# s-esposito/MonoGS

Hardware: AMD Instinct MI355X
Metric: rasteriser fwd+bwd Mpix/s @1080p (higher is better)
Workload: dtype f32; 1 GPU; C5: 2000000 Gaussians, 1920x1080, fwd+bwd, seeded synthetic map (SURVEY.md 8d), one keyframe per GPU; gaussians=2000000, width=1920, height=1080, settle_steps=60, instance_count=device-side (capacity mode, overflow checked), parallelism=keyframe-per-gpu x1

## Files before the change

monogs_amd/csrc/blend.hip:

```cpp
#include "common.h"
#include "tile_sort.h"

#include <type_traits>


namespace mgs {

#ifdef BS_TRACE
static unsigned long long* g_trace_fwd = nullptr;
static unsigned long long* g_trace_bwd = nullptr;
static unsigned long long g_trace_bwd_records = 0;
#define BS_STAMP(v) asm volatile("s_memrealtime %0\n\ts_waitcnt lgkmcnt(0)" : "=s"(v) :: "memory")
#endif

__device__ __forceinline__ uint32_t bcast(uint32_t v, int lane) {
    return (uint32_t)__builtin_amdgcn_readlane((int)v, lane);
}

constexpr int MGS_WG_WAVES = 4;
#define MGS_TILE_WAVE(ntiles_, tile_, wave_, ws_)                                                   \
    const int tile_ = (int)blockIdx.x, wave_ = __builtin_amdgcn_readfirstlane((int)(threadIdx.x >> 6)), ws_ = wave_; \
    if (tile_ >= (ntiles_)) return;
struct BlendArgs {
#ifdef BS_TRACE
    unsigned long long* trace;
#endif
    const float4* __restrict__ rec;
    const uint32_t* __restrict__ point_list;
    const uint2* __restrict__ ranges;
    const float* __restrict__ bg;
    unsigned long long* fwd_masks;
    int W, H, gx;
};
__device__ __forceinline__ size_t fwd_mask_word(uint32_t range_x, int tile, int wave) {
    return ((size_t)(range_x / WAVE) + (size_t)tile) * 4 + (size_t)wave;
}

__device__ __forceinline__ bool quadrant_hit(const float4 c , const float4 n ,
                                             float qx0, float qy0, unsigned long long alive) {
    const float x0 = qx0 - 0.05f - c.x, x1 = qx0 + (float)(SUB - 1) + 0.05f - c.x;
    const float y0 = qy0 - 0.05f - c.y, y1 = qy0 + (float)(SUB - 1) + 0.05f - c.y;
    if (c.z < 0.f) return false;
    if (!((c.z >= x0) && (-c.z <= x1) && (c.w >= y0) && (-c.w <= y1))) return false;
    {
        const int ix0 = (int)fminf(8.f, fmaxf(0.f, ceilf(-x0 - c.z - 0.06f))), ix1 = (int)fminf(7.f, fmaxf(-1.f, floorf(-x0 + c.z + 0.06f)));
        const int iy0 = (int)fminf(8.f, fmaxf(0.f, ceilf(-y0 - c.w - 0.06f))), iy1 = (int)fminf(7.f, fmaxf(-1.f, floorf(-y0 + c.w + 0.06f)));
        if (ix0 > ix1 || iy0 > iy1) return false;
        const unsigned long long cols = (unsigned long long)((0xFFu >> (7 - ix1)) & (0xFFu << ix0) & 0xFFu) * 0x0101010101010101ull;
        const unsigned long long rows = (~0ull >> (8 * (7 - iy1))) & (~0ull << (8 * iy0));
        if ((cols & rows & alive) == 0ull) return false;
    }
    if (x0 <= 0.f && x1 >= 0.f && y0 <= 0.f && y1 >= 0.f) return true;
    if (!(n.x > 0.f) || !(n.z > 0.f)) return true;
    const float rby = -n.y * __builtin_amdgcn_rcpf(n.z), rbx = -n.y * __builtin_amdgcn_rcpf(n.x);
    auto edge_x = [&](float xe) {
        const float t = fminf(y1, fmaxf(y0, rby * xe));
        return n.x * xe * xe + 2.f * n.y * xe * t + n.z * t * t;
    };
    auto edge_y = [&](float ye) {
        const float t = fminf(x1, fmaxf(x0, rbx * ye));
        return n.x * t * t + 2.f * n.y * t * ye + n.z * ye * ye;
    };
    const float qmin = fminf(fminf(edge_x(x0), edge_x(x1)), fminf(edge_y(y0), edge_y(y1)));
    return qmin <= 1.02f;
}

struct Rec {
    float px, py, ca, cb, cc, op, r, g, b, z;
};
__device__ __forceinline__ Rec fetch(const BlendArgs& a, uint32_t gid_uniform) {
    const const_float_p p = MGS_CONST(reinterpret_cast<const float*>(a.rec)) + (size_t)gid_uniform * REC_FLOATS;
    return Rec{p[R_X], p[R_Y], p[R_CA], p[R_CB], p[R_CC], p[R_OPAC], p[R_R], p[R_G], p[R_B], p[R_DEPTH]};
}

template <bool TOUCH>
__device__ __forceinline__ void blend_one(unsigned long long& live, unsigned long long& mask, float& T, uint32_t& last, float& C0, float& C1, float& C2,
                                      float& D, const Rec& g, float power, float alpha, uint32_t pos, int j,
                                      int& touched_cnt) {
    const float test_T = T * (1.f - alpha);
    float w;
    int cnt;
    if (TOUCH) {
        asm volatile(
            "s_mov_b64 exec, %[live]\n\t"
            "v_cmpx_nlt_f32_e32 vcc, 0, %[power]\n\t"
            "v_cmpx_ngt_f32_e32 vcc, %[amin], %[alpha]\n\t"
            "v_cmp_gt_f32_e32 vcc, %[tmin], %[tt]\n\t"
            "s_andn2_b64 exec, exec, vcc\n\t"
            "s_andn2_b64 %[live], %[live], vcc\n\t"
            "s_cselect_b64 %[mask], %[mask], 0\n\t"
            "v_mul_f32_e32 %[w], %[alpha], %[T]\n\t"
            "v_mov_b32_e32 %[T], %[tt]\n\t"
            "v_mov_b32_e32 %[last], %[pos]\n\t"
            "v_cmp_lt_f32_e32 vcc, 0.5, %[tt]\n\t"
            "v_fmac_f32_e32 %[C0], %[cr], %[w]\n\t"
            "v_fmac_f32_e32 %[C1], %[cg], %[w]\n\t"
            "s_bcnt1_i32_b64 %[cnt], vcc\n\t"
            "s_mov_b32 m0, %[j]\n\t"
            "v_fmac_f32_e32 %[C2], %[cb], %[w]\n\t"
            "v_fmac_f32_e32 %[D], %[cz], %[w]\n\t"
            "s_mov_b64 exec, -1\n\t"
            "v_writelane_b32 %[tc], %[cnt], m0\n\t"
            : [live] "+s"(live), [mask] "+s"(mask), [T] "+v"(T), [last] "+v"(last), [C0] "+v"(C0), [C1] "+v"(C1), [C2] "+v"(C2), [D] "+v"(D),
              [w] "=&v"(w), [cnt] "=&s"(cnt), [tc] "+v"(touched_cnt)
            : [power] "v"(power), [alpha] "v"(alpha), [tt] "v"(test_T), [amin] "s"(1.0f / 255.0f), [tmin] "s"(0.0001f),
              [pos] "s"(pos), [cr] "v"(g.r), [cg] "v"(g.g), [cb] "v"(g.b), [cz] "v"(g.z), [j] "s"(j)
            : "vcc", "scc", "m0");
    } else {
        asm volatile(
            "s_mov_b64 exec, %[live]\n\t"
            "v_cmpx_nlt_f32_e32 vcc, 0, %[power]\n\t"
            "v_cmpx_ngt_f32_e32 vcc, %[amin], %[alpha]\n\t"
            "v_cmp_gt_f32_e32 vcc, %[tmin], %[tt]\n\t"
            "s_andn2_b64 exec, exec, vcc\n\t"
            "s_andn2_b64 %[live], %[live], vcc\n\t"
            "s_cselect_b64 %[mask], %[mask], 0\n\t"
            "v_mul_f32_e32 %[w], %[alpha], %[T]\n\t"
            "v_mov_b32_e32 %[T], %[tt]\n\t"
            "v_mov_b32_e32 %[last], %[pos]\n\t"
            "v_fmac_f32_e32 %[C0], %[cr], %[w]\n\t"
            "v_fmac_f32_e32 %[C1], %[cg], %[w]\n\t"
            "v_fmac_f32_e32 %[C2], %[cb], %[w]\n\t"
            "v_fmac_f32_e32 %[D], %[cz], %[w]\n\t"
            "s_mov_b64 exec, -1\n\t"
            : [live] "+s"(live), [mask] "+s"(mask), [T] "+v"(T), [last] "+v"(last), [C0] "+v"(C0), [C1] "+v"(C1), [C2] "+v"(C2), [D] "+v"(D),
              [w] "=&v"(w)
            : [power] "v"(power), [alpha] "v"(alpha), [tt] "v"(test_T), [amin] "s"(1.0f / 255.0f), [tmin] "s"(0.0001f),
              [pos] "s"(pos), [cr] "v"(g.r), [cg] "v"(g.g), [cb] "v"(g.b), [cz] "v"(g.z)
            : "vcc", "scc");
    }
}

template <bool SORT>
__global__ void __launch_bounds__(256) blend_forward_kernel(BlendArgs a, float* __restrict__ out_color,
                                                            float* __restrict__ out_depth,
                                                            float* __restrict__ out_opacity,
                                                            float* __restrict__ final_T,
                                                            uint32_t* __restrict__ n_contrib,
                                                            int32_t* __restrict__ n_touched,
                                                            uint2* ranges_rw ,
                                                            const uint32_t* __restrict__ sort_err,
                                                            uint32_t* __restrict__ status, TileSortArgs ts,
                                                            const unsigned long long* __restrict__ prepare ,
                                                            int P, int lines_per_tile ) {
    MGS_TILE_WAVE(a.gx * ((a.H + TILE - 1) / TILE), tile, wave, ws)
    if (prepare) {
        float* const acc = reinterpret_cast<float*>((uintptr_t)MGS_CONST_U64(prepare)[1]);
        if (acc) {
            const int first = tile * lines_per_tile;
            const int n4 = 4 * min(lines_per_tile, P - first);
            float4* const base = reinterpret_cast<float4*>(acc + (size_t)first * GRAD_FLOATS);
            for (int i = (int)threadIdx.x; i < n4; i += 256) base[i] = make_float4(0.f, 0.f, 0.f, 0.f);
        }
    }
    const int tx = tile % a.gx, ty = tile / a.gx;
    const int lane = threadIdx.x & 63;
    const bool first_of_tile = wave == 0 && lane == 0;
    const int qx0i = tx * TILE + (wave & 1) * SUB, qy0i = ty * TILE + (wave >> 1) * SUB;
    const int pxi = qx0i + (lane & 7), pyi = qy0i + (lane >> 3);
    const bool inside = pxi < a.W && pyi < a.H;
    const float pxf = (float)pxi, pyf = (float)pyi;
    const float qx0 = (float)qx0i, qy0 = (float)qy0i;
    uint2 range = ranges_rw[tile];
    const uint2 range_raw = range;
    const bool sort_bad = sort_err != nullptr && radix_failed(sort_err) != 0u;
    {
        if (sort_bad && tile == 0 && first_of_tile && status) atomicOr(status, (uint32_t)MGS_STATUS_TILE_SORT_TIMEOUT);
        if (sort_bad || range.x >= range.y) {
            range = make_uint2(0u, 0u);
            if (first_of_tile) ranges_rw[tile] = range;
        }
    }

    float T = 1.f, C0 = 0.f, C1 = 0.f, C2 = 0.f, D = 0.f;
    uint32_t last = 0;
    unsigned long long live = __builtin_amdgcn_ballot_w64(inside);
#ifdef BS_TRACE
    unsigned long long tr0;
    BS_STAMP(tr0);
#endif

    uint32_t gid_n = 0;
    float4 box_n = make_float4(0.f, 0.f, -1.f, -1.f), ell_n = make_float4(0.f, 0.f, 0.f, 0.f);
    __shared__ __attribute__((aligned(16))) float4 s_queue[MGS_WG_WAVES][WAVE][3];
    __shared__ uint32_t s_list[TDS_CAP], s_wsum[TDS_WAVES], s_red[2 * TDS_WAVES];
    static_assert(sizeof(s_queue) == sizeof(uint32_t) * (TDS_CAP + TDS_WAVES * TDS_RADIX), "sort scratch = record queue");
    bool list_in_lds = false;
    if constexpr (SORT) {
        uint32_t* const s_k = reinterpret_cast<uint32_t*>(&s_queue[0][0][0]);
        const uint32_t n_lds = tile_depth_sort(ts, range_raw, sort_bad,
                                               TdsLds{s_k, s_list, reinterpret_cast<uint32_t (*)[TDS_RADIX]>(s_k + TDS_CAP),
                                                      s_wsum, s_red});
        list_in_lds = n_lds != 0u && n_lds == range.y - range.x;
        if (!list_in_lds) __syncthreads();
    }
    float4 c1_n = make_float4(0.f, 0.f, 0.f, 0.f), c2_n = c1_n;
    float4* const my_entry = &s_queue[ws][lane][0];
    const uint32_t q_base = (uint32_t)__builtin_amdgcn_readfirstlane((int)(uint32_t)(uintptr_t)&s_queue[ws][0][0]);
    auto prefetch = [&](uint32_t i) {
        gid_n = 0;
        box_n = make_float4(0.f, 0.f, -1.f, -1.f);
        if (i < range.y) {
            if constexpr (SORT) gid_n = list_in_lds ? s_list[i - range.x] : ts.vals[i];
            else gid_n = a.point_list[i];
            box_n = a.rec[(size_t)gid_n * 4];
            ell_n = a.rec[(size_t)gid_n * 4 + 3];
            c1_n = a.rec[(size_t)gid_n * 4 + 1];
            c2_n = a.rec[(size_t)gid_n * 4 + 2];
        }
    };
    auto walk_step = [&](auto touch_tag, uint32_t base, uint32_t gid_l, unsigned long long mask) {
        int touched_cnt = 0;
        while (mask) {
            const int j = __builtin_ctzll(mask);
            mask &= ~(1ull << j);
            typedef float qv2 __attribute__((ext_vector_type(2)));
            typedef float qv4 __attribute__((ext_vector_type(4)));
            qv2 e0;
            qv4 e1, e2;
            {
                const uint32_t ad = q_base + (uint32_t)j * 48u;
                asm volatile("ds_read_b64 %0, %3\n\tds_read_b128 %1, %3 offset:16\n\tds_read_b128 %2, %3 offset:32"
                             : "=&v"(e0), "=&v"(e1), "=&v"(e2) : "v"(ad) : "memory");
            }
            asm volatile("s_waitcnt lgkmcnt(2)" : "+v"(e0));
            float dx = e0[0] - pxf, dy = e0[1] - pyf;
            asm volatile("s_waitcnt lgkmcnt(1)" : "+v"(e1), "+v"(dx), "+v"(dy));
            const float power = dx * (e1[0] * dx + e1[1] * dy) + (e1[2] * dy) * dy;
            float alpha = fminf(0.99f, e1[3] * __builtin_amdgcn_exp2f(power));
            asm volatile("s_waitcnt lgkmcnt(0)" : "+v"(e2), "+v"(alpha));
            const Rec g{e0[0], e0[1], e1[0], e1[1], e1[2], e1[3], e2[0], e2[1], e2[2], e2[3]};
            blend_one<decltype(touch_tag)::value>(live, mask, T, last, C0, C1, C2, D, g, power, alpha,
                                                  (base - range.x) + (uint32_t)j + 1u, j, touched_cnt);
        }
        if (decltype(touch_tag)::value && touched_cnt != 0) atomicAdd(n_touched + gid_l, touched_cnt);
    };
    unsigned long long* const mask_row = a.fwd_masks + fwd_mask_word((uint32_t)__builtin_amdgcn_readfirstlane((int)range.x), tile, wave);
    uint32_t mask_off = 0;
    if (range.x < range.y) prefetch(range.x + lane);
    for (uint32_t base = range.x; base < range.y && live != 0ull; base += WAVE) {
        const uint32_t gid_l = gid_n;
        const float4 c = box_n, el = ell_n;
        my_entry[0] = c; my_entry[1] = c1_n; my_entry[2] = c2_n;
        prefetch(base + WAVE + lane);
        const unsigned long long mask = __builtin_amdgcn_ballot_w64(quadrant_hit(c, el, qx0, qy0, live));
        if ((live & __builtin_amdgcn_ballot_w64(T > 0.5f)) != 0ull) walk_step(std::true_type{}, base, gid_l, mask);
        else walk_step(std::false_type{}, base, gid_l, mask);
        if (__builtin_amdgcn_inverse_ballot_w64(1ull))
            asm volatile("global_store_dwordx2 %0, %1, %2" ::"v"(mask_off), "v"(mask), "s"(mask_row) : "memory");
        mask_off += 4u * (uint32_t)sizeof(unsigned long long);
    }
#ifdef BS_TRACE
    if (a.trace) {
        unsigned long long tr1;
        BS_STAMP(tr1);
        const unsigned hw = __builtin_amdgcn_s_getreg((31 << 11) | 4), xcc = __builtin_amdgcn_s_getreg((31 << 11) | 20);
        if (lane == 0) {
            unsigned long long* o = a.trace + ((size_t)tile * 4 + wave) * 4;
            o[0] = tr0; o[1] = tr1; o[2] = (unsigned long long)hw | ((unsigned long long)xcc << 32); o[3] = range.y - range.x;
        }
    }
#endif
    if (inside) {
        const size_t pix = (size_t)pyi * a.W + pxi, HW = (size_t)a.H * a.W;
        final_T[pix] = T;
        n_contrib[pix] = last;
        out_color[pix] = C0 + T * a.bg[0];
        out_color[HW + pix] = C1 + T * a.bg[1];
        out_color[2 * HW + pix] = C2 + T * a.bg[2];
        out_depth[pix] = D;
        out_opacity[pix] = 1.f - T;
    }
}

static BlendArgs make_args(const mgs_camera& cam, const GeometryState& g, const BinningState& b,
                           const ImageState& img) {
    BlendArgs a;
#ifdef BS_TRACE
    a.trace = nullptr;
#endif
    a.rec = reinterpret_cast<const float4*>(g.rec);
    a.point_list = b.vals_sorted;
    a.ranges = img.ranges;
    a.bg = cam.bg;
    a.fwd_masks = b.fwd_masks;
    a.W = cam.image_width;
    a.H = cam.image_height;
    a.gx = tiles_x(a.W);
    return a;
}

int launch_blend_forward(const mgs_camera& cam, const GeometryState& g, const BinningState& b,
                         const ImageState& img, float* out_color, float* out_depth, float* out_opacity,
                         int32_t* n_touched, const uint32_t* sort_err, uint32_t* status, const TileSortArgs* tile_sort,
                         int P, hipStream_t s) {
    BlendArgs a = make_args(cam, g, b, img);
#ifdef BS_TRACE
    a.trace = g_trace_fwd;
#endif
    const int ntiles = a.gx * tiles_y(a.H);
    if (ntiles == 0) return 0;
    const dim3 grid(ntiles), block(256);
    const TileSortArgs ts = tile_sort ? *tile_sort : TileSortArgs{};
    const unsigned long long* const prepare = P > 0 ? g.prepare : nullptr;
    const int lines_per_tile = (P + ntiles - 1) / ntiles;
    if (tile_sort)
        hipLaunchKernelGGL(blend_forward_kernel<true>, grid, block, 0, s, a, out_color, out_depth,
                           out_opacity, img.final_T, img.n_contrib, n_touched, img.ranges, sort_err, status, ts, prepare, P,
                           lines_per_tile);
    else
        hipLaunchKernelGGL(blend_forward_kernel<false>, grid, block, 0, s, a, out_color, out_depth,
                           out_opacity, img.final_T, img.n_contrib, n_touched, img.ranges, sort_err, status, ts, prepare, P,
                           lines_per_tile);
    MGS_HIP(hipGetLastError());
    return 0;
}


__device__ __forceinline__ float swap32_add(float x, float y) {
    auto r = __builtin_amdgcn_permlane32_swap(__float_as_uint(x), __float_as_uint(y), false, false);
    return __uint_as_float(r[0]) + __uint_as_float(r[1]);
}
__device__ __forceinline__ float swap16_add(float x, float y) {
    auto r = __builtin_amdgcn_permlane16_swap(__float_as_uint(x), __float_as_uint(y), false, false);
    return __uint_as_float(r[0]) + __uint_as_float(r[1]);
}
template <int XOR>
__device__ __forceinline__ float swz_add(float v) {
    return v + __int_as_float(__builtin_amdgcn_ds_swizzle(__float_as_int(v), 0x001F | (XOR << 10)));
}
__device__ __forceinline__ float row_sum_all(float v) {
    v = swz_add<1>(v);
    v = swz_add<2>(v);
    v = swz_add<4>(v);
    v = swz_add<8>(v);
    return v;
}
__device__ __forceinline__ int reduce10_slot(int lane) {
    const int row = lane >> 4, pos = lane & 15;
    if (pos == 15) return row == 0 ? 0 : row == 1 ? 2 : row == 2 ? 1 : 3;
    if (pos == 0) return row == 0 ? 4 : row == 1 ? 6 : row == 2 ? 5 : 7;
    if (pos == 1) return row == 0 ? 8 : row == 2 ? 9 : -1;
    return -1;
}
__device__ __forceinline__ float reduce10(float a0, float a1, float a2, float a3, float a4, float a5, float a6,
                                          float a7, float a8, float a9, int lane) {
    const float b0 = swap32_add(a0, a1), b1 = swap32_add(a2, a3), b2 = swap32_add(a4, a5);
    const float b3 = swap32_add(a6, a7), b4 = swap32_add(a8, a9);
    float c0 = swap16_add(b0, b1);
    float c1 = swap16_add(b2, b3);
    float c2 = swz_add<16>(b4);
    c0 = row_sum_all(c0);
    c1 = row_sum_all(c1);
    c2 = row_sum_all(c2);
    const int pos = lane & 15;
    return pos == 15 ? c0 : (pos == 0 ? c1 : c2);
}

__device__ __forceinline__ int reduce6_slot(int lane) {
    const int row = lane >> 4, pos = lane & 15;
    if (pos == 15) return row == 0 ? G_SX : row == 1 ? G_SXX : row == 2 ? G_SY : G_SXY;
    if (pos == 0) return row == 0 ? G_SYY : row == 2 ? G_DDEPTH : -1;
    return -1;
}
__device__ __forceinline__ float reduce6(float a0, float a1, float a2, float a3, float a4, float a5, int lane) {
    const float b0 = swap32_add(a0, a1), b1 = swap32_add(a2, a3), b2 = swap32_add(a4, a5);
    float c0 = swap16_add(b0, b1);
    float c1 = swz_add<16>(b2);
    c0 = row_sum_all(c0);
    c1 = row_sum_all(c1);
    return (lane & 15) == 15 ? c0 : c1;
}

__device__ __forceinline__ uint32_t wave_max_u32(uint32_t v) {
#pragma unroll
    for (int o = 32; o > 0; o >>= 1) v = max(v, (uint32_t)__shfl_xor((int)v, o, 64));
    return v;
}

template <bool POSE_ONLY>
__global__ void __launch_bounds__(256) blend_backward_kernel(BlendArgs a, int ntiles,
                                                             const float* __restrict__ final_T,
                                                             const uint32_t* __restrict__ n_contrib,
                                                             const float* __restrict__ dL_dcolor,
                                                             const float* __restrict__ dL_ddepth,
                                                             float* __restrict__ grad_acc) {
    const int wave = threadIdx.x >> 6, lane = threadIdx.x & 63;
    const int tile = (int)blockIdx.x;
    if (tile >= ntiles) return;
    const int tx = tile % a.gx, ty = tile / a.gx;
    const uint2 range = a.ranges[tile];
    if (range.y <= range.x) return;
    const size_t HW = (size_t)a.H * a.W;
    const float bg0 = a.bg[0], bg1 = a.bg[1], bg2 = a.bg[2];

    const int qx0i = tx * TILE + (wave & 1) * SUB, qy0i = ty * TILE + (wave >> 1) * SUB;
    const int pxi = qx0i + (lane & 7), pyi = qy0i + (lane >> 3);
    const bool inside = pxi < a.W && pyi < a.H;
    const size_t pix = (size_t)pyi * a.W + pxi;
    const float pxf = (float)pxi, pyf = (float)pyi, qx0 = (float)qx0i, qy0 = (float)qy0i;
    const float T_final = inside ? final_T[pix] : 0.f;
    const uint32_t last = inside ? n_contrib[pix] : 0u;
    const float g0 = inside ? dL_dcolor[pix] : 0.f;
    const float g1 = inside ? dL_dcolor[HW + pix] : 0.f;
    const float g2 = inside ? dL_dcolor[2 * HW + pix] : 0.f;
    const float gd = inside ? dL_ddepth[pix] : 0.f;
    const float bgT = -T_final * (bg0 * g0 + bg1 * g1 + bg2 * g2);
    float T = T_final, Bk = 0.f;
    const uint32_t maxc = wave_max_u32(last);
    if (maxc == 0) return;
    const uint32_t end = range.x + maxc;

    const int slot = POSE_ONLY ? reduce6_slot(lane) : reduce10_slot(lane);
    const uint32_t slot_bytes = slot < 0 ? 0u : (uint32_t)slot * 4u;

    uint32_t gid_n = 0;
    float4 box_n = make_float4(0.f, 0.f, -1.f, -1.f), ell_n = make_float4(0.f, 0.f, 0.f, 0.f);
    auto prefetch = [&](int b) {
        gid_n = 0;
        box_n = make_float4(0.f, 0.f, -1.f, -1.f);
        const uint32_t i = range.x + (uint32_t)b * WAVE + lane;
        if (b >= 0 && i < end) {
            gid_n = a.point_list[i];
            box_n = a.rec[(size_t)gid_n * 4];
            ell_n = a.rec[(size_t)gid_n * 4 + 3];
        }
    };
    prefetch((int)((maxc - 1) / WAVE));
    for (int b = (int)((maxc - 1) / WAVE); b >= 0; --b) {
        const uint32_t gid_l = gid_n;
        const float4 c = box_n, el = ell_n;
        prefetch(b - 1);
        const unsigned long long alive = __builtin_amdgcn_ballot_w64(last >= (uint32_t)b * WAVE + 1u);
        unsigned long long mask = __builtin_amdgcn_ballot_w64(quadrant_hit(c, el, qx0, qy0, alive));
        const int rel_last = (int)last - (int)((uint32_t)b * WAVE + 1u);
        while (mask) {
            const int j = 63 - __builtin_clzll(mask);
            mask &= ~(1ull << j);
            const uint32_t gid = bcast(gid_l, j);
            const Rec g = fetch(a, gid);
            const float dx = g.px - pxf, dy = g.py - pyf;
            const float power = dx * (g.ca * dx + g.cb * dy) + (g.cc * dy) * dy;
            const float G = __builtin_amdgcn_exp2f(power);
            const float alpha = fminf(0.99f, g.op * G);
            const bool act = (j <= rel_last) && !(power > 0.f) && !(alpha < 1.0f / 255.0f);
            if (__builtin_amdgcn_ballot_w64(act) == 0ull) continue;
            const float a_eff = act ? alpha : 0.f;
            const float inv = __builtin_amdgcn_rcpf(1.f - a_eff);
            const float Tn = T * inv;
            const float qq = __builtin_fmaf(g.z, gd, __builtin_fmaf(g.b, g2, __builtin_fmaf(g.g, g1, g.r * g0)));
            const float diff = qq - Bk;
            const float dL_dalpha = diff * Tn + bgT * inv;
            Bk = Bk + a_eff * diff;
            T = Tn;
            const float w = a_eff * Tn;
            const float h = act ? G * dL_dalpha : 0.f;
            const float hx = h * dx, hy = h * dy;
            const float s_x = hx, s_y = hy, s_xx = hx * dx, s_xy = hx * dy, s_yy = hy * dy, s_h = h;
            const float s_r = w * g0, s_g = w * g1, s_b = w * g2, s_z = w * gd;
            const float m = POSE_ONLY ? reduce6(s_x, s_y, s_xx, s_xy, s_yy, s_z, lane)
                                      : reduce10(s_x, s_y, s_xx, s_xy, s_yy, s_h, s_r, s_g, s_b, s_z, lane);
            float* const line = grad_acc + (size_t)gid * GRAD_FLOATS;
            if (slot >= 0) asm volatile("global_atomic_add_f32 %0, %1, %2" ::"v"(slot_bytes), "v"(m), "s"(line) : "memory");
        }
    }
}

constexpr int BT_SLOTS = 4;
constexpr int BS_STRIDE = 272;
constexpr int BS_W_OFF = 1280;
constexpr int BS_META_OFF = BS_W_OFF + BT_SLOTS * BS_STRIDE;
__device__ __forceinline__ int bt_slot10(int t) {
    const int bank = t >> 2, m = t & 3;
    if (m == 0) return bank == 3 ? 0 : bank == 1 ? 1 : bank == 2 ? 2 : 3;
    if (m == 1) return bank == 3 ? 4 : bank == 1 ? 5 : bank == 2 ? 6 : 7;
    if (m == 2) return bank == 3 ? 8 : bank == 1 ? 9 : -1;
    return -1;
}
__device__ __forceinline__ int bt_slot6(int t) {
    const int bank = t >> 2, m = t & 3;
    if (m == 0) return bank == 3 ? G_SX : bank == 1 ? G_SY : bank == 2 ? G_SXX : G_SXY;
    if (m == 1) return bank == 3 ? G_SYY : bank == 1 ? G_DDEPTH : -1;
    return -1;
}
__device__ __forceinline__ float reduce_rows10(float v0, float v1, float v2, float v3, float v4, float v5, float v6,
                                               float v7, float v8, float v9, unsigned long long m1, unsigned long long m2) {
    float a0, a1, a2, a3, a4;
    asm volatile(
        "s_nop 1\n\t"
        "v_add_f32_dpp %0, %5, %5 row_ror:8 row_mask:0xf bank_mask:0xc\n\t"
        "v_add_f32_dpp %1, %7, %7 row_ror:8 row_mask:0xf bank_mask:0xc\n\t"
        "v_add_f32_dpp %2, %9, %9 row_ror:8 row_mask:0xf bank_mask:0xc\n\t"
        "v_add_f32_dpp %3, %11, %11 row_ror:8 row_mask:0xf bank_mask:0xc\n\t"
        "v_add_f32_dpp %4, %13, %13 row_ror:8 row_mask:0xf bank_mask:0xc\n\t"
        "v_add_f32_dpp %0, %6, %6 row_ror:8 row_mask:0xf bank_mask:0x3\n\t"
        "v_add_f32_dpp %1, %8, %8 row_ror:8 row_mask:0xf bank_mask:0x3\n\t"
        "v_add_f32_dpp %2, %10, %10 row_ror:8 row_mask:0xf bank_mask:0x3\n\t"
        "v_add_f32_dpp %3, %12, %12 row_ror:8 row_mask:0xf bank_mask:0x3\n\t"
        "v_add_f32_dpp %4, %14, %14 row_ror:8 row_mask:0xf bank_mask:0x3\n\t"
        "v_add_f32_dpp %5, %0, %0 row_half_mirror row_mask:0xf bank_mask:0xa\n\t"
        "v_add_f32_dpp %6, %2, %2 row_half_mirror row_mask:0xf bank_mask:0xa\n\t"
        "v_add_f32_dpp %5, %1, %1 row_half_mirror row_mask:0xf bank_mask:0x5\n\t"
        "v_add_f32_dpp %6, %3, %3 row_half_mirror row_mask:0xf bank_mask:0x5\n\t"
        "v_add_f32_dpp %7, %4, %4 row_half_mirror row_mask:0xf bank_mask:0xf\n\t"
        "v_add_f32_dpp %0, %5, %5 quad_perm:[2,3,0,1] row_mask:0xf bank_mask:0xf\n\t"
        "v_add_f32_dpp %1, %6, %6 quad_perm:[2,3,0,1] row_mask:0xf bank_mask:0xf\n\t"
        "v_add_f32_dpp %2, %7, %7 quad_perm:[2,3,0,1] row_mask:0xf bank_mask:0xf\n\t"
        "v_add_f32_dpp %5, %0, %0 quad_perm:[1,0,3,2] row_mask:0xf bank_mask:0xf\n\t"
        "v_add_f32_dpp %6, %1, %1 quad_perm:[1,0,3,2] row_mask:0xf bank_mask:0xf\n\t"
        "v_add_f32_dpp %7, %2, %2 quad_perm:[1,0,3,2] row_mask:0xf bank_mask:0xf\n\t"
        : "=&v"(a0), "=&v"(a1), "=&v"(a2), "=&v"(a3), "=&v"(a4), "+v"(v0), "+v"(v1), "+v"(v2), "+v"(v3), "+v"(v4), "+v"(v5),
          "+v"(v6), "+v"(v7), "+v"(v8), "+v"(v9));
    const float r12 = __builtin_amdgcn_inverse_ballot_w64(m1) ? v1 : v2;
    return __builtin_amdgcn_inverse_ballot_w64(m2) ? v0 : r12;
}
__device__ __forceinline__ float reduce_rows6(float v0, float v1, float v2, float v3, float v4, float v5,
                                              unsigned long long m2) {
    float a0, a1, a2;
    asm volatile(
        "s_nop 1\n\t"
        "v_add_f32_dpp %0, %3, %3 row_ror:8 row_mask:0xf bank_mask:0xc\n\t"
        "v_add_f32_dpp %1, %5, %5 row_ror:8 row_mask:0xf bank_mask:0xc\n\t"
        "v_add_f32_dpp %2, %7, %7 row_ror:8 row_mask:0xf bank_mask:0xc\n\t"
        "v_add_f32_dpp %0, %4, %4 row_ror:8 row_mask:0xf bank_mask:0x3\n\t"
        "v_add_f32_dpp %1, %6, %6 row_ror:8 row_mask:0xf bank_mask:0x3\n\t"
        "v_add_f32_dpp %2, %8, %8 row_ror:8 row_mask:0xf bank_mask:0x3\n\t"
        "v_add_f32_dpp %3, %0, %0 row_half_mirror row_mask:0xf bank_mask:0xa\n\t"
        "v_add_f32_dpp %3, %1, %1 row_half_mirror row_mask:0xf bank_mask:0x5\n\t"
        "v_add_f32_dpp %4, %2, %2 row_half_mirror row_mask:0xf bank_mask:0xf\n\t"
        "s_nop 1\n\t"
        "v_add_f32_dpp %0, %3, %3 quad_perm:[2,3,0,1] row_mask:0xf bank_mask:0xf\n\t"
        "v_add_f32_dpp %1, %4, %4 quad_perm:[2,3,0,1] row_mask:0xf bank_mask:0xf\n\t"
        "s_nop 0\n\t"
        "v_add_f32_dpp %3, %0, %0 quad_perm:[1,0,3,2] row_mask:0xf bank_mask:0xf\n\t"
        "v_add_f32_dpp %4, %1, %1 quad_perm:[1,0,3,2] row_mask:0xf bank_mask:0xf\n\t"
        : "=&v"(a0), "=&v"(a1), "=&v"(a2), "+v"(v0), "+v"(v1), "+v"(v2), "+v"(v3), "+v"(v4), "+v"(v5));
    return __builtin_amdgcn_inverse_ballot_w64(m2) ? v0 : v1;
}

struct __attribute__((aligned(16))) BtMetaRec { float x, y; uint32_t g; };
struct BtLane {
    const float* fac;
    const float* pix;
    const BtMetaRec* meta;
    int lane;
    float qx0, qy0;
    uint32_t slot_bytes;
    unsigned long long m_out, m_q0, m_q1;
    float* grad_acc;
    int qxi = 0, qyi = 0;
};
template <bool POSE_ONLY, bool WIDE_META = false>
__device__ __forceinline__ void bt_flush(const BtLane L, int n) {
// ... 711 lines not shown
```

Baseline: 2967 Mpix/s.

## Deepen forward blend prefetch pipeline and fuse per-splat alpha math into asm

Restructures the forward blend walk so the Gaussian list index is fetched two batches ahead and the records one batch ahead. The loop is specialised at compile time on whether the sorted list lives in LDS and on the touch phase. Since T only decreases, the touch-counting loop is left permanently once no live pixel has T above 0.5, instead of being re-checked per batch. The per-splat LDS read, conic evaluation, exp, alpha clamp and blend now sit in one inline-asm block with explicit lgkmcnt waits. The aim is to hide global-load latency and remove per-splat scheduling overhead, at the cost of more live registers and more hand-written asm to maintain.

```diff
diff --git a/monogs_amd/csrc/blend.hip b/monogs_amd/csrc/blend.hip
--- a/monogs_amd/csrc/blend.hip
+++ b/monogs_amd/csrc/blend.hip
@@ -73,62 +73,95 @@
     return Rec{p[R_X], p[R_Y], p[R_CA], p[R_CB], p[R_CC], p[R_OPAC], p[R_R], p[R_G], p[R_B], p[R_DEPTH]};
 }
 
+#define MGS_TRIP_ALPHA                                                                                                  \
+    "s_waitcnt lgkmcnt(2)\n\t"                                                                                          \
+    "v_sub_f32_e32 %[dx], %[x], %[px]\n\t"                                                                              \
+    "v_sub_f32_e32 %[dy], %[y], %[py]\n\t"                                                                              \
+    "s_waitcnt lgkmcnt(1)\n\t"                                                                                          \
+    "v_mul_f32_e32 %[t], %[dy], %[cb]\n\t"                                                                              \
+    "v_fmac_f32_e32 %[t], %[dx], %[ca]\n\t"                                                                             \
+    "v_mul_f32_e32 %[u], %[dy], %[cc]\n\t"                                                                              \
+    "v_mul_f32_e32 %[t], %[dx], %[t]\n\t"                                                                               \
+    "v_fmac_f32_e32 %[t], %[dy], %[u]\n\t"                                                                              \
+    "v_exp_f32_e32 %[dx], %[t]\n\t"                                                                                     \
+    "s_mov_b64 exec, %[live]\n\t"                                                                                       \
+    "v_mul_f32_e32 %[dx], %[op], %[dx]\n\t"                                                                             \
+    "v_min_f32_e32 %[dx], 0x3f7d70a4, %[dx]\n\t"                                                                        \
+    "v_sub_f32_e32 %[u], 1.0, %[dx]\n\t"                                                                                \
+    "v_mul_f32_e32 %[u], %[T], %[u]\n\t"                                                                                \
+    "v_cmpx_nlt_f32_e32 vcc, 0, %[t]\n\t"                                                                               \
+    "v_cmpx_ngt_f32_e32 vcc, %[amin], %[dx]\n\t"                                                                        \
+    "v_cmp_gt_f32_e32 vcc, %[tmin], %[u]\n\t"                                                                           \
+    "s_andn2_b64 exec, exec, vcc\n\t"                                                                                   \
+    "s_andn2_b64 %[live], %[live], vcc\n\t"                                                                             \
+    "s_cselect_b64 %[mask], %[mask], 0\n\t"                                                                             \
+    "v_mul_f32_e32 %[dy], %[dx], %[T]\n\t"                                                                              \
+    "v_mov_b32_e32 %[T], %[u]\n\t"                                                                                      \
+    "v_mov_b32_e32 %[last], %[pos]\n\t"
 template <bool TOUCH>
-__device__ __forceinline__ void blend_one(unsigned long long& live, unsigned long long& mask, float& T, uint32_t& last, float& C0, float& C1, float& C2,
-                                      float& D, const Rec& g, float power, float alpha, uint32_t pos, int j,
-                                      int& touched_cnt) {
-    const float test_T = T * (1.f - alpha);
-    float w;
-    int cnt;
+__device__ __forceinline__ void blend_trip(unsigned long long& live, unsigned long long& mask, float& T, uint32_t& last, float& C0, float& C1,
+                                           float& C2, float& D, float pxf, float pyf, uint32_t vq, uint32_t pos0, int& touched_cnt) {
+    typedef float qv2 __attribute__((ext_vector_type(2)));
+    typedef float qv4 __attribute__((ext_vector_type(4)));
+    int j;
+    uint32_t ad;
+    qv2 e0;
+    qv4 e1, e2;
+    asm volatile(
+        "s_ff1_i32_b64 %[j], %[mask]\n\t"
+        "s_bitset0_b64 %[mask], %[j]\n\t"
+        "v_mad_u32_u24 %[ad], %[j], 48, %[vq]\n\t"
+        "ds_read_b64 %[e0], %[ad]\n\t"
+        "ds_read_b128 %[e1], %[ad] offset:16\n\t"
+        "ds_read_b128 %[e2], %[ad] offset:32\n\t"
+        : [j] "=&s"(j), [mask] "+s"(mask), [ad] "=&v"(ad), [e0] "=&v"(e0), [e1] "=&v"(e1), [e2] "=&v"(e2)
+        : [vq] "v"(vq)
+        : "memory");
+    const uint32_t pos = pos0 + (uint32_t)j;
+    float dx, dy, t, u;
     if (TOUCH) {
+        int cnt;
         asm volatile(
-            "s_mov_b64 exec, %[live]\n\t"
-            "v_cmpx_nlt_f32_e32 vcc, 0, %[power]\n\t"
-            "v_cmpx_ngt_f32_e32 vcc, %[amin], %[alpha]\n\t"
-            "v_cmp_gt_f32_e32 vcc, %[tmin], %[tt]\n\t"
-            "s_andn2_b64 exec, exec, vcc\n\t"
-            "s_andn2_b64 %[live], %[live], vcc\n\t"
-            "s_cselect_b64 %[mask], %[mask], 0\n\t"
-            "v_mul_f32_e32 %[w], %[alpha], %[T]\n\t"
-            "v_mov_b32_e32 %[T], %[tt]\n\t"
-            "v_mov_b32_e32 %[last], %[pos]\n\t"
-            "v_cmp_lt_f32_e32 vcc, 0.5, %[tt]\n\t"
-            "v_fmac_f32_e32 %[C0], %[cr], %[w]\n\t"
-            "v_fmac_f32_e32 %[C1], %[cg], %[w]\n\t"
+            "s_mov_b32 m0, %[j]\n\t"
+            MGS_TRIP_ALPHA
+            "v_cmp_lt_f32_e32 vcc, 0.5, %[u]\n\t"
+            "s_waitcnt lgkmcnt(0)\n\t"
+            "v_fmac_f32_e32 %[C0], %[r], %[dy]\n\t"
+            "v_fmac_f32_e32 %[C1], %[g], %[dy]\n\t"
             "s_bcnt1_i32_b64 %[cnt], vcc\n\t"
-            "s_mov_b32 m0, %[j]\n\t"
-            "v_fmac_f32_e32 %[C2], %[cb], %[w]\n\t"
-            "v_fmac_f32_e32 %[D], %[cz], %[w]\n\t"
+            "v_fmac_f32_e32 %[C2], %[b], %[dy]\n\t"
+            "v_fmac_f32_e32 %[D], %[z], %[dy]\n\t"
             "s_mov_b64 exec, -1\n\t"
             "v_writelane_b32 %[tc], %[cnt], m0\n\t"
             : [live] "+s"(live), [mask] "+s"(mask), [T] "+v"(T), [last] "+v"(last), [C0] "+v"(C0), [C1] "+v"(C1), [C2] "+v"(C2), [D] "+v"(D),
-              [w] "=&v"(w), [cnt] "=&s"(cnt), [tc] "+v"(touched_cnt)
-            : [power] "v"(power), [alpha] "v"(alpha), [tt] "v"(test_T), [amin] "s"(1.0f / 255.0f), [tmin] "s"(0.0001f),
-              [pos] "s"(pos), [cr] "v"(g.r), [cg] "v"(g.g), [cb] "v"(g.b), [cz] "v"(g.z), [j] "s"(j)
+              [dx] "=&v"(dx), [dy] "=&v"(dy), [t] "=&v"(t), [u] "=&v"(u), [cnt] "=&s"(cnt),
+              [tc] "+v"(touched_cnt)
+            : [px] "v"(pxf), [py] "v"(pyf), [x] "v"(e0[0]), [y] "v"(e0[1]), [ca] "v"(e1[0]), [cb] "v"(e1[1]), [cc] "v"(e1[2]), [op] "v"(e1[3]), [r] "v"(e2[0]), [g] "v"(e2[1]), [b] "v"(e2[2]), [z] "v"(e2[3]), [pos] "s"(pos),
+              [amin] "s"(1.0f / 255.0f), [tmin] "s"(0.0001f), [j] "s"(j)
             : "vcc", "scc", "m0");
     } else {
         asm volatile(
-            "s_mov_b64 exec, %[live]\n\t"
-            "v_cmpx_nlt_f32_e32 vcc, 0, %[power]\n\t"
-            "v_cmpx_ngt_f32_e32 vcc, %[amin], %[alpha]\n\t"
-            "v_cmp_gt_f32_e32 vcc, %[tmin], %[tt]\n\t"
-            "s_andn2_b64 exec, exec, vcc\n\t"
-            "s_andn2_b64 %[live], %[live], vcc\n\t"
-            "s_cselect_b64 %[mask], %[mask], 0\n\t"
-            "v_mul_f32_e32 %[w], %[alpha], %[T]\n\t"
-            "v_mov_b32_e32 %[T], %[tt]\n\t"
-            "v_mov_b32_e32 %[last], %[pos]\n\t"
-            "v_fmac_f32_e32 %[C0], %[cr], %[w]\n\t"
-            "v_fmac_f32_e32 %[C1], %[cg], %[w]\n\t"
-            "v_fmac_f32_e32 %[C2], %[cb], %[w]\n\t"
-            "v_fmac_f32_e32 %[D], %[cz], %[w]\n\t"
+            MGS_TRIP_ALPHA
+            "s_waitcnt lgkmcnt(0)\n\t"
+            "v_fmac_f32_e32 %[C0], %[r], %[dy]\n\t"
+            "v_fmac_f32_e32 %[C1], %[g], %[dy]\n\t"
+            "v_fmac_f32_e32 %[C2], %[b], %[dy]\n\t"
+            "v_fmac_f32_e32 %[D], %[z], %[dy]\n\t"
             "s_mov_b64 exec, -1\n\t"
             : [live] "+s"(live), [mask] "+s"(mask), [T] "+v"(T), [last] "+v"(last), [C0] "+v"(C0), [C1] "+v"(C1), [C2] "+v"(C2), [D] "+v"(D),
-              [w] "=&v"(w)
-            : [power] "v"(power), [alpha] "v"(alpha), [tt] "v"(test_T), [amin] "s"(1.0f / 255.0f), [tmin] "s"(0.0001f),
-              [pos] "s"(pos), [cr] "v"(g.r), [cg] "v"(g.g), [cb] "v"(g.b), [cz] "v"(g.z)
+              [dx] "=&v"(dx), [dy] "=&v"(dy), [t] "=&v"(t), [u] "=&v"(u)
+            : [px] "v"(pxf), [py] "v"(pyf), [x] "v"(e0[0]), [y] "v"(e0[1]), [ca] "v"(e1[0]), [cb] "v"(e1[1]), [cc] "v"(e1[2]), [op] "v"(e1[3]), [r] "v"(e2[0]), [g] "v"(e2[1]), [b] "v"(e2[2]), [z] "v"(e2[3]), [pos] "s"(pos),
+              [amin] "s"(1.0f / 255.0f), [tmin] "s"(0.0001f)
             : "vcc", "scc");
     }
+}
+
+__device__ __forceinline__ uint32_t lds_u32(const uint32_t* base, uint32_t i) {
+#if defined(__HIP_DEVICE_COMPILE__)
+    return ((const __attribute__((address_space(3))) uint32_t*)base)[i];
+#else
+    return base[i];
+#endif
 }
 
 template <bool SORT>
@@ -180,8 +213,7 @@
     BS_STAMP(tr0);
 #endif
 
-    uint32_t gid_n = 0;
-    float4 box_n = make_float4(0.f, 0.f, -1.f, -1.f), ell_n = make_float4(0.f, 0.f, 0.f, 0.f);
+    const uint32_t rx = (uint32_t)__builtin_amdgcn_readfirstlane((int)range.x), ry = (uint32_t)__builtin_amdgcn_readfirstlane((int)range.y);
     __shared__ __attribute__((aligned(16))) float4 s_queue[MGS_WG_WAVES][WAVE][3];
     __shared__ uint32_t s_list[TDS_CAP], s_wsum[TDS_WAVES], s_red[2 * TDS_WAVES];
     static_assert(sizeof(s_queue) == sizeof(uint32_t) * (TDS_CAP + TDS_WAVES * TDS_RADIX), "sort scratch = record queue");
@@ -191,64 +223,71 @@
         const uint32_t n_lds = tile_depth_sort(ts, range_raw, sort_bad,
                                                TdsLds{s_k, s_list, reinterpret_cast<uint32_t (*)[TDS_RADIX]>(s_k + TDS_CAP),
                                                       s_wsum, s_red});
-        list_in_lds = n_lds != 0u && n_lds == range.y - range.x;
+        list_in_lds = __builtin_amdgcn_readfirstlane((int)(n_lds != 0u && n_lds == ry - rx)) != 0;
         if (!list_in_lds) __syncthreads();
     }
-    float4 c1_n = make_float4(0.f, 0.f, 0.f, 0.f), c2_n = c1_n;
     float4* const my_entry = &s_queue[ws][lane][0];
     const uint32_t q_base = (uint32_t)__builtin_amdgcn_readfirstlane((int)(uint32_t)(uintptr_t)&s_queue[ws][0][0]);
-    auto prefetch = [&](uint32_t i) {
-        gid_n = 0;
-        box_n = make_float4(0.f, 0.f, -1.f, -1.f);
-        if (i < range.y) {
-            if constexpr (SORT) gid_n = list_in_lds ? s_list[i - range.x] : ts.vals[i];
-            else gid_n = a.point_list[i];
-            box_n = a.rec[(size_t)gid_n * 4];
-            ell_n = a.rec[(size_t)gid_n * 4 + 3];
-            c1_n = a.rec[(size_t)gid_n * 4 + 1];
-            c2_n = a.rec[(size_t)gid_n * 4 + 2];
-        }
+    uint32_t vq = q_base;
+    asm volatile("" : "+v"(vq));
+    struct StepSet {
+        uint32_t gid;
+        float4 box, ell, c1, c2;
     };
-    auto walk_step = [&](auto touch_tag, uint32_t base, uint32_t gid_l, unsigned long long mask) {
-        int touched_cnt = 0;
-        while (mask) {
-            const int j = __builtin_ctzll(mask);
-            mask &= ~(1ull << j);
-            typedef float qv2 __attribute__((ext_vector_type(2)));
-            typedef float qv4 __attribute__((ext_vector_type(4)));
-            qv2 e0;
-            qv4 e1, e2;
-            {
-                const uint32_t ad = q_base + (uint32_t)j * 48u;
-                asm volatile("ds_read_b64 %0, %3\n\tds_read_b128 %1, %3 offset:16\n\tds_read_b128 %2, %3 offset:32"
-                             : "=&v"(e0), "=&v"(e1), "=&v"(e2) : "v"(ad) : "memory");
-            }
-            asm volatile("s_waitcnt lgkmcnt(2)" : "+v"(e0));
-            float dx = e0[0] - pxf, dy = e0[1] - pyf;
-            asm volatile("s_waitcnt lgkmcnt(1)" : "+v"(e1), "+v"(dx), "+v"(dy));
-            const float power = dx * (e1[0] * dx + e1[1] * dy) + (e1[2] * dy) * dy;
-            float alpha = fminf(0.99f, e1[3] * __builtin_amdgcn_exp2f(power));
-            asm volatile("s_waitcnt lgkmcnt(0)" : "+v"(e2), "+v"(alpha));
-            const Rec g{e0[0], e0[1], e1[0], e1[1], e1[2], e1[3], e2[0], e2[1], e2[2], e2[3]};
-            blend_one<decltype(touch_tag)::value>(live, mask, T, last, C0, C1, C2, D, g, power, alpha,
-                                                  (base - range.x) + (uint32_t)j + 1u, j, touched_cnt);
-        }
-        if (decltype(touch_tag)::value && touched_cnt != 0) atomicAdd(n_touched + gid_l, touched_cnt);
+    StepSet cur, nxt;
+    uint32_t idx_n = 0;
+    auto fetch_index = [&](auto lds_tag, uint32_t i) -> uint32_t {
+        const uint32_t ic = min(i, ry - 1u);
+        if constexpr (SORT) {
+            if constexpr (decltype(lds_tag)::value) return lds_u32(s_list, ic - rx);
+            else return ts.vals[ic];
+        } else {
+            return a.point_list[ic];
+        }
     };
-    unsigned long long* const mask_row = a.fwd_masks + fwd_mask_word((uint32_t)__builtin_amdgcn_readfirstlane((int)range.x), tile, wave);
+    auto fetch_records = [&](StepSet& n, uint32_t i, uint32_t idx) {
+        n.gid = idx;
+        n.box = a.rec[(size_t)idx * 4];
+        n.ell = a.rec[(size_t)idx * 4 + 3];
+        n.c1 = a.rec[(size_t)idx * 4 + 1];
+        n.c2 = a.rec[(size_t)idx * 4 + 2];
+        n.box.z = i < ry ? n.box.z : -1.f;
+    };
+    unsigned long long* const mask_row = a.fwd_masks + fwd_mask_word(rx, tile, wave);
     uint32_t mask_off = 0;
-    if (range.x < range.y) prefetch(range.x + lane);
-    for (uint32_t base = range.x; base < range.y && live != 0ull; base += WAVE) {
-        const uint32_t gid_l = gid_n;
-        const float4 c = box_n, el = ell_n;
-        my_entry[0] = c; my_entry[1] = c1_n; my_entry[2] = c2_n;
-        prefetch(base + WAVE + lane);
-        const unsigned long long mask = __builtin_amdgcn_ballot_w64(quadrant_hit(c, el, qx0, qy0, live));
-        if ((live & __builtin_amdgcn_ballot_w64(T > 0.5f)) != 0ull) walk_step(std::true_type{}, base, gid_l, mask);
-        else walk_step(std::false_type{}, base, gid_l, mask);
-        if (__builtin_amdgcn_inverse_ballot_w64(1ull))
-            asm volatile("global_store_dwordx2 %0, %1, %2" ::"v"(mask_off), "v"(mask), "s"(mask_row) : "memory");
-        mask_off += 4u * (uint32_t)sizeof(unsigned long long);
+    uint32_t base = rx;
+    auto steps = [&](auto touch_tag, auto lds_tag) {
+        constexpr bool TOUCH = decltype(touch_tag)::value;
+        for (; base < ry && live != 0ull; base += WAVE) {
+            if (TOUCH && (live & __builtin_amdgcn_ballot_w64(T > 0.5f)) == 0ull) return;
+            const uint32_t i_n = base + WAVE + lane;
+            my_entry[0] = cur.box; my_entry[1] = nxt.c1; my_entry[2] = nxt.c2;
+            const uint32_t gid_l = cur.gid;
+            const float4 c = cur.box, el = cur.ell;
+            fetch_records(nxt, i_n, idx_n);
+            idx_n = fetch_index(lds_tag, i_n + WAVE);
+            unsigned long long mask = __builtin_amdgcn_ballot_w64(quadrant_hit(c, el, qx0, qy0, live));
+            const unsigned long long mask_all = mask;
+            int touched_cnt = 0;
+            while (mask) blend_trip<TOUCH>(live, mask, T, last, C0, C1, C2, D, pxf, pyf, vq, base - rx + 1u, touched_cnt);
+            if (TOUCH && touched_cnt != 0) atomicAdd(n_touched + gid_l, touched_cnt);
+            if (__builtin_amdgcn_inverse_ballot_w64(1ull))
+                asm volatile("global_store_dwordx2 %0, %1, %2" ::"v"(mask_off), "v"(mask_all), "s"(mask_row) : "memory");
+            mask_off += 4u * (uint32_t)sizeof(unsigned long long);
+            asm volatile("" ::"v"(nxt.ell.w));
+            cur.gid = nxt.gid; cur.box = nxt.box; cur.ell = nxt.ell;
+        }
+    };
+    auto walk = [&](auto lds_tag) {
+        fetch_records(nxt, rx + lane, fetch_index(lds_tag, rx + lane));
+        idx_n = fetch_index(lds_tag, rx + WAVE + lane);
+        cur.gid = nxt.gid; cur.box = nxt.box; cur.ell = nxt.ell;
+        steps(std::true_type{}, lds_tag);
+        steps(std::false_type{}, lds_tag);
+    };
+    if (rx < ry && live != 0ull) {
+        if (SORT && list_in_lds) walk(std::true_type{});
+        else walk(std::false_type{});
     }
 #ifdef BS_TRACE
     if (a.trace) {
```

Measured after the change: 2988 Mpix/s (median of 6 runs). Within noise of the previous version (+0.7%).
